# walexi/gnn.cpp

Hardware: AMD Instinct MI355X
Metric: GCN-layer edges/sec (fwd+bwd: X.W^T + normalized-adjacency SpMM + their gradients) (higher is better)
Workload: dtype f32

## Files before the change

### gnn.cpp_amd/csrc/gnnx_gemm.hip

```cpp
#include <atomic>

#include "gnnx_common.h"

using namespace gnnx;

namespace {

typedef float f32x16 __attribute__((ext_vector_type(16)));

struct GemmArgs {
    int64_t M, N, K;
    const float *A;
    int64_t lda;
    const float *B;
    int64_t ldb;
    float *C;
    int64_t ldc;
    float alpha, beta;
    int64_t k_per_split;
    float *slab;
    int64_t k_pairs;
};

template <int BM_, int BN_, int BK_, int WM_, int WN_>
struct Cfg {
    static constexpr int BM = BM_, BN = BN_, BK = BK_, WM = WM_, WN = WN_;
    static constexpr int NT = 64 * WM * WN;
    static constexpr int TM = BM / WM / 32, TN = BN / WN / 32;
    static constexpr int ld_a(bool kc) { return kc ? BM + 2 : BM + 4; }
    static constexpr int ld_b(bool kc) { return kc ? BN + 2 : BN + 4; }
    static constexpr size_t lds_bytes(bool a_kc, bool b_kc) { return sizeof(float) * 2 * BK * (ld_a(a_kc) + ld_b(b_kc)); }
    static constexpr int A_VECS = BM * BK / 4 / NT;
    static constexpr int B_VECS = BN * BK / 4 / NT;
    static_assert(A_VECS >= 1 && B_VECS >= 1, "tile too small for the thread count");
};

template <bool KC, bool VEC, int ROWS, int BK, int NT, int NV>
__device__ __forceinline__ void load_tile(float (&reg)[NV * 4], const float *base, int64_t ld, int64_t r0, int64_t rmax,
                                          int64_t k0, int64_t kmax, int tid)
{
#pragma unroll
    for (int i = 0; i < NV; i++) {
        const int idx = tid + i * NT;
        int64_t r, k;
        if constexpr (KC) {
            r = r0 + idx / (BK / 4);
            k = k0 + (idx % (BK / 4)) * 4;
            const int64_t rc = r < rmax ? r : rmax - 1;
            if constexpr (VEC) {
                const float4 v = *reinterpret_cast<const float4 *>(base + rc * ld + (k < kmax ? k : 0));
                reg[4 * i + 0] = v.x;
                reg[4 * i + 1] = v.y;
                reg[4 * i + 2] = v.z;
                reg[4 * i + 3] = v.w;
            } else {
#pragma unroll
                for (int j = 0; j < 4; j++) reg[4 * i + j] = base[rc * ld + ((k + j) < kmax ? (k + j) : 0)];
            }
        } else {
            k = k0 + idx / (ROWS / 4);
            r = r0 + (idx % (ROWS / 4)) * 4;
            const int64_t kc = k < kmax ? k : kmax - 1;
            if constexpr (VEC) {
                const float4 v = *reinterpret_cast<const float4 *>(base + kc * ld + (r < rmax ? r : 0));
                reg[4 * i + 0] = v.x;
                reg[4 * i + 1] = v.y;
                reg[4 * i + 2] = v.z;
                reg[4 * i + 3] = v.w;
            } else {
#pragma unroll
                for (int j = 0; j < 4; j++) reg[4 * i + j] = base[kc * ld + ((r + j) < rmax ? (r + j) : 0)];
            }
        }
    }
}

template <bool KC, bool MASK, int ROWS, int BK, int NT, int NV, int LD>
__device__ __forceinline__ void store_tile_impl(float *lds, const float (&reg)[NV * 4], int tid, int64_t r0, int64_t rmax,
                                                int64_t k0, int64_t kmax)
{
#pragma unroll
    for (int i = 0; i < NV; i++) {
        const int idx = tid + i * NT;
        if constexpr (KC) {
            const int r = idx / (BK / 4), k = (idx % (BK / 4)) * 4;
#pragma unroll
            for (int j = 0; j < 4; j++) {
                float v = reg[4 * i + j];
                if constexpr (MASK) v = (r0 + r < rmax && k0 + k + j < kmax) ? v : 0.f;
                lds[(k + j) * LD + r] = v;
            }
        } else {
            const int k = idx / (ROWS / 4), r = (idx % (ROWS / 4)) * 4;
            float v[4];
#pragma unroll
            for (int j = 0; j < 4; j++) {
                v[j] = reg[4 * i + j];
                if constexpr (MASK) v[j] = (k0 + k < kmax && r0 + r + j < rmax) ? v[j] : 0.f;
            }
            if constexpr (LD % 4 == 0) {
                *reinterpret_cast<float4 *>(lds + k * LD + r) = make_float4(v[0], v[1], v[2], v[3]);
            } else {
#pragma unroll
                for (int j = 0; j < 4; j++) lds[k * LD + r + j] = v[j];
            }
        }
    }
}

template <bool KC, int ROWS, int BK, int NT, int NV, int LD>
__device__ __forceinline__ void store_tile(float *lds, const float (&reg)[NV * 4], int tid, bool full, int64_t r0, int64_t rmax,
                                           int64_t k0, int64_t kmax)
{
    if (full) store_tile_impl<KC, false, ROWS, BK, NT, NV, LD>(lds, reg, tid, r0, rmax, k0, kmax);
    else store_tile_impl<KC, true, ROWS, BK, NT, NV, LD>(lds, reg, tid, r0, rmax, k0, kmax);
}

template <class C, bool A_KC, bool B_KC, bool VEC_A, bool VEC_B>
__global__ __launch_bounds__(C::NT) void gemm_kernel(GemmArgs g)
{
    constexpr int BM = C::BM, BN = C::BN, BK = C::BK, NT = C::NT, TM = C::TM, TN = C::TN;
    constexpr int LDA = C::ld_a(A_KC), LDB = C::ld_b(B_KC);
    extern __shared__ __attribute__((aligned(16))) float lds_raw[];
    const int tid = threadIdx.x;
    const int lane = tid & 63, wave = tid >> 6;
    const int wm = wave / C::WN, wn = wave % C::WN;
    const int64_t m0 = (int64_t)blockIdx.y * BM, n0 = (int64_t)blockIdx.x * BN;
    const int64_t kbeg = (int64_t)blockIdx.z * g.k_per_split;
    const int64_t kend = kbeg + g.k_per_split < g.K ? kbeg + g.k_per_split : g.K;
    const bool full_mn = m0 + BM <= g.M && n0 + BN <= g.N;

    f32x16 acc[TM][TN];
#pragma unroll
    for (int i = 0; i < TM; i++)
#pragma unroll
        for (int j = 0; j < TN; j++)
#pragma unroll
            for (int r = 0; r < 16; r++) acc[i][j][r] = 0.f;

    constexpr int STORE_AT = (BK * 3 / 4) & ~1;
    float ra[C::A_VECS * 4], rb[C::B_VECS * 4];
    int buf = 0;
    if (kbeg < kend) {
        const bool full = full_mn && kbeg + BK <= kend;
        load_tile<A_KC, VEC_A, BM, BK, NT, C::A_VECS>(ra, g.A, g.lda, m0, g.M, kbeg, kend, tid);
        load_tile<B_KC, VEC_B, BN, BK, NT, C::B_VECS>(rb, g.B, g.ldb, n0, g.N, kbeg, kend, tid);
        store_tile<A_KC, BM, BK, NT, C::A_VECS, LDA>(lds_raw, ra, tid, full, m0, g.M, kbeg, kend);
        store_tile<B_KC, BN, BK, NT, C::B_VECS, LDB>(lds_raw + 2 * BK * LDA, rb, tid, full, n0, g.N, kbeg, kend);
    }
    __syncthreads();
    for (int64_t k0 = kbeg; k0 < kend; k0 += BK) {
        const bool more = k0 + BK < kend;
// ... 103 lines not shown
        for (int i = 0; i < C::A_VECS; i++) {
            const float4 v = *reinterpret_cast<const float4 *>(abase + offa[i]);
            ra[4 * i + 0] = v.x; ra[4 * i + 1] = v.y; ra[4 * i + 2] = v.z; ra[4 * i + 3] = v.w;
        }
#pragma unroll
        for (int i = 0; i < C::B_VECS; i++) {
            const float4 v = *reinterpret_cast<const float4 *>(bbase + offb[i]);
            rb[4 * i + 0] = v.x; rb[4 * i + 1] = v.y; rb[4 * i + 2] = v.z; rb[4 * i + 3] = v.w;
        }
    };
    auto stash = [&](int b) {
        store_tile_impl<true, false, BM, BK, NT, C::A_VECS, LDA>(lds_raw + b * BK * LDA, ra, tid, 0, 0, 0, 0);
        store_tile_impl<B_KC, false, BN, BK, NT, C::B_VECS, LDB>(lds_raw + 2 * BK * LDA + b * BK * LDB, rb, tid, 0, 0, 0, 0);
    };

    f32x16 acc[TM][TN];
    constexpr int STORE_AT = (BK * 3 / 4) & ~1;
    int buf = 0;
    int64_t mt = blockIdx.y;
    if (mt < m_tiles) {
        load(mt, 0);
        stash(0);
    }
    __syncthreads();
    for (; mt < m_tiles; mt += gridDim.y) {
        const int64_t mt_next = mt + gridDim.y;
#pragma unroll
        for (int i = 0; i < TM; i++)
#pragma unroll
            for (int j = 0; j < TN; j++)
#pragma unroll
                for (int r = 0; r < 16; r++) acc[i][j][r] = 0.f;
        for (int64_t k0 = 0; k0 < g.K; k0 += BK) {
            const bool last_k = k0 + BK >= g.K;
            const bool more = !last_k || mt_next < m_tiles;
            if (more) load(last_k ? mt_next : mt, last_k ? 0 : k0 + BK);
            const float *As = lds_raw + buf * BK * LDA + wm * (BM / C::WM) + (lane & 31) + (lane >> 5) * LDA;
            const float *Bs = lds_raw + 2 * BK * LDA + buf * BK * LDB + wn * (BN / C::WN) + (lane & 31) + (lane >> 5) * LDB;
            float a[2][TM], b[2][TN];
#pragma unroll
            for (int i = 0; i < TM; i++) a[0][i] = As[32 * i];
#pragma unroll
            for (int j = 0; j < TN; j++) b[0][j] = Bs[32 * j];
#pragma unroll
            for (int kk = 0; kk < BK; kk += 2) {
                const int cur = (kk >> 1) & 1, nxt = cur ^ 1;
                if (kk + 2 < BK) {
#pragma unroll
                    for (int i = 0; i < TM; i++) a[nxt][i] = As[(kk + 2) * LDA + 32 * i];
#pragma unroll
                    for (int j = 0; j < TN; j++) b[nxt][j] = Bs[(kk + 2) * LDB + 32 * j];
                }
                __builtin_amdgcn_sched_barrier(0);
#pragma unroll
                for (int i = 0; i < TM; i++)
#pragma unroll
                    for (int j = 0; j < TN; j++)
                        acc[i][j] = __builtin_amdgcn_mfma_f32_32x32x2f32(a[cur][i], b[cur][j], acc[i][j], 0, 0, 0);
                __builtin_amdgcn_sched_barrier(0);
                if (kk == STORE_AT && more) {
                    stash(buf ^ 1);
                    __builtin_amdgcn_sched_barrier(0);
                }
            }
            __syncthreads();
            buf ^= 1;
        }
        float *cbase = g.C + mt * BM * g.ldc + n0;
#pragma unroll
        for (int i = 0; i < TM; i++)
#pragma unroll
            for (int j = 0; j < TN; j++)
#pragma unroll
                for (int r = 0; r < 16; r++)
                    (cbase + (int64_t)(i * 32 + (r & 3) + 8 * (r >> 2)) * g.ldc + j * 32)[offc] = g.alpha * acc[i][j][r];
    }
}

typedef __attribute__((address_space(3))) void gemm_lds_void_t;
typedef float gemm_f32x4 __attribute__((ext_vector_type(4)));
typedef float gemm_f32x4acc __attribute__((ext_vector_type(4)));

template <int OFF>
__device__ __forceinline__ void lds_read_b32(float &dst, uint32_t addr)
{
    static_assert(OFF >= 0 && OFF < 65536, "ds_read offset is a 16-bit unsigned immediate");
    asm volatile("ds_read_b32 %0, %1 offset:%2" : "=v"(dst) : "v"(addr), "i"(OFF) : "memory");
}

template <int WM_, int WN_>
struct DmaGeo {
    static constexpr int WM = WM_, WN = WN_, NW = WM * WN, NT = 64 * NW;
    static constexpr int BM = 64 * WM, BN = 64 * WN, BK = 32;
    static constexpr int SLOTS = BK / 4;
    static constexpr int A_ROW_BYTES = BK * 4, A_BLOCK_BYTES = 16 * A_ROW_BYTES;
    static constexpr int A_ROWS_PER_INSTR = 1024 / A_ROW_BYTES;
    static constexpr int a_xor(int row) { return (row / 2) % SLOTS; }
    static constexpr int A_STAGE_BYTES = BM * BK * 4;
    static constexpr int A_PER_WAVE = (BM / A_ROWS_PER_INSTR) / NW;
    static constexpr int rows_per_instr(int width) { return 256 / width; }
    static constexpr int KPIECE_BYTES = 272 * 4;
    static constexpr int kstage_bytes(int width) { return (BK / rows_per_instr(width)) * KPIECE_BYTES; }
    static constexpr int kgroup_off(int width, int KG)
    {
        return rows_per_instr(width) == 1 ? 4 * KG * KPIECE_BYTES : (4 * (KG % (BK / 8))) * KPIECE_BYTES + (KG / (BK / 8)) * 512;
    }
    static constexpr int krow_of(int width, int I, int lane) { return rows_per_instr(width) == 1 ? I : I + (BK / 2) * (lane / 32); }
    static constexpr int B_STAGE_BYTES = kstage_bytes(BN);
    static constexpr int B_PIECE_BYTES = KPIECE_BYTES;
    static constexpr int B_PER_WAVE = (BK / rows_per_instr(BN)) / NW;
    static constexpr int STAGES_BYTES = 2 * A_STAGE_BYTES + 2 * B_STAGE_BYTES;
    static constexpr int EP_EXTRA = A_PER_WAVE + B_PER_WAVE >= 4 ? 0 : 4 - A_PER_WAVE - B_PER_WAVE;
    static constexpr int LDS_BYTES = STAGES_BYTES + NW * EP_EXTRA * 1024;
    static_assert(A_PER_WAVE >= 1 && B_PER_WAVE >= 1, "too many wavefronts for the operand tile");
};

template <class GEO, int STAGE_ID, int KG>
__device__ __forceinline__ void dma2_read_group(float (&a)[4], float (&b)[4], const uint32_t (&ak)[GEO::SLOTS], uint32_t bk)
{
    constexpr int SA = STAGE_ID * GEO::A_STAGE_BYTES, BLK = GEO::A_BLOCK_BYTES;
    lds_read_b32<SA + 0 * BLK>(a[0], ak[KG]);
    lds_read_b32<SA + 1 * BLK>(a[1], ak[KG]);
    lds_read_b32<SA + 2 * BLK>(a[2], ak[KG]);
    lds_read_b32<SA + 3 * BLK>(a[3], ak[KG]);
    constexpr int SB = STAGE_ID * GEO::B_STAGE_BYTES + GEO::kgroup_off(GEO::BN, KG);
    lds_read_b32<SB + 0 * 64>(b[0], bk);
    lds_read_b32<SB + 1 * 64>(b[1], bk);
    lds_read_b32<SB + 2 * 64>(b[2], bk);
    lds_read_b32<SB + 3 * 64>(b[3], bk);
}

#define GNNX_DMA2_WAIT(N, set)                                                                                                   \
    asm volatile("s_waitcnt lgkmcnt(" #N ")" : "+v"(a[set][0]), "+v"(a[set][1]), "+v"(a[set][2]), "+v"(a[set][3]), "+v"(b[set][0]), \
                 "+v"(b[set][1]), "+v"(b[set][2]), "+v"(b[set][3])::"memory")
#define GNNX_DMA2_MFMA(set)                                                                                \
    _Pragma("unroll") for (int i_ = 0; i_ < 4; i_++) _Pragma("unroll") for (int j_ = 0; j_ < 4; j_++)      \
        acc[i_][j_] = __builtin_amdgcn_mfma_f32_16x16x4f32(b[set][j_], a[set][i_], acc[i_][j_], 0, 0, 0)
#define GNNX_DMA2_STEP(ST, KG, cur, nxt)                                  \
    dma2_read_group<GEO, ST, KG + 1>(a[nxt], b[nxt], ak, bk);            \
    GNNX_DMA2_WAIT(8, cur);                                               \
    GNNX_DMA2_MFMA(cur)
#define GNNX_DMA2_KTILE(ST)                                               \
    dma2_read_group<GEO, ST, 0>(a[0], b[0], ak, bk);                     \
    GNNX_DMA2_STEP(ST, 0, 0, 1);                                          \
    GNNX_DMA2_STEP(ST, 1, 1, 0);                                          \
    GNNX_DMA2_STEP(ST, 2, 0, 1);                                          \
    GNNX_DMA2_STEP(ST, 3, 1, 0);                                          \
    GNNX_DMA2_STEP(ST, 4, 0, 1);                                          \
    GNNX_DMA2_STEP(ST, 5, 1, 0);                                          \
    GNNX_DMA2_STEP(ST, 6, 0, 1);                                          \
    GNNX_DMA2_WAIT(0, 1);                                                 \
    GNNX_DMA2_MFMA(1)

__device__ __forceinline__ void dma_16B(uint32_t voff_bytes, const float *sbase, uint32_t lds_dst)
{
    uint32_t keep;
    asm volatile("s_nop 4\n\ts_mov_b32 %0, m0\n\ts_mov_b32 m0, %3\n\ts_nop 0\n\tglobal_load_lds_dwordx4 %1, %2\n\ts_mov_b32 m0, %0"
                 : "=&s"(keep) : "v"(voff_bytes), "s"(sbase), "s"(lds_dst) : "memory");
}

enum class Epi { kPlain, kReluColsum, kBnSums, kBf16, kSendSlots };

constexpr bool epi_covers_rows(Epi e) { return e == Epi::kPlain || e == Epi::kSendSlots; }

struct GemmFuse {
    const float *ymask;
    int64_t ldy;
    float *colsum_partial;
    const int32_t *slots;
};

template <int WM_, int WN_, Epi EPI, bool NG>
__global__ __launch_bounds__(64 * WM_ * WN_, 1) void gemm_dma_kernel(GemmArgs g, GemmFuse fu, int64_t m_tiles)
{
    using GEO = DmaGeo<WM_, WN_>;
    constexpr int BM = GEO::BM, BN = GEO::BN, BK = GEO::BK, NW = GEO::NW;
    constexpr int APW = GEO::A_PER_WAVE, BPW = GEO::B_PER_WAVE;
    extern __shared__ __attribute__((aligned(16))) float lds_raw[];
    const int tid = threadIdx.x;
    const int lane = tid & 63;
    const int wave = __builtin_amdgcn_readfirstlane(tid >> 6);
    const int wm = wave / GEO::WN, wn = wave % GEO::WN;
    const int q = lane >> 4, r16 = lane & 15;
    const int64_t n0 = (int64_t)blockIdx.x * BN;
    const uint32_t lds0 = (uint32_t)(uintptr_t)(gemm_lds_void_t *)lds_raw;
    constexpr uint32_t B0 = 2 * GEO::A_STAGE_BYTES;

    uint32_t offa[APW], offb[BPW], pa[APW], pb[BPW];
#pragma unroll
    for (int u = 0; u < APW; u++) {
        const int row = GEO::A_ROWS_PER_INSTR * (wave + NW * u) + lane / GEO::SLOTS;
        const int kg = (lane % GEO::SLOTS) ^ GEO::a_xor(row);
        offa[u] = (uint32_t)(row * g.lda + 4 * kg) * 4u;
        pa[u] = lds0 + (uint32_t)((wave + NW * u) * 1024);
    }
#pragma unroll
    for (int u = 0; u < BPW; u++) {
        constexpr int RPI = GEO::rows_per_instr(BN), LPR = 64 / RPI;
        const int krow = GEO::krow_of(BN, wave + NW * u, lane);
        offb[u] = (uint32_t)(krow * g.ldb + 4 * (lane % LPR)) * 4u;
        pb[u] = lds0 + B0 + (uint32_t)((wave + NW * u) * GEO::B_PIECE_BYTES);
    }
    const float *bcol = g.B + n0;
    const int64_t n_left = g.N - n0;
    const bool okb = !NG || 4 * (lane % (64 / GEO::rows_per_instr(BN))) + 4 <= n_left;
    const bool okc = !NG || wn * 64 + 4 * (lane & 15) + 4 <= n_left;
    const int64_t last_row0 = g.M - BM;
    auto row0_of = [&](int64_t mt) { return mt * BM <= last_row0 ? mt * BM : last_row0; };
    auto issue = [&](int stage, int64_t mt, int64_t k0) {
        const float *abase = g.A + row0_of(mt) * g.lda + k0;
        const float *bbase = bcol + k0 * g.ldb;
#pragma unroll
        for (int u = 0; u < (APW > BPW ? APW : BPW); u++) {
            if (u < APW) dma_16B(offa[u < APW ? u : 0], abase, pa[u < APW ? u : 0] + stage * GEO::A_STAGE_BYTES);
            if (u < BPW && okb) dma_16B(offb[u < BPW ? u : 0], bbase, pb[u < BPW ? u : 0] + stage * GEO::B_STAGE_BYTES);
        }
    };
    uint32_t ak[GEO::SLOTS];
    {
        const int row = wm * 64 + r16;
        const uint32_t xa = (uint32_t)(GEO::a_xor(row) << 4);
#pragma unroll
        for (int kg = 0; kg < GEO::SLOTS; kg++) ak[kg] = lds0 + (uint32_t)(row * GEO::A_ROW_BYTES + 4 * q) + (((uint32_t)kg << 4) ^ xa);
    }
    const uint32_t bk = lds0 + B0 + (uint32_t)(q * GEO::KPIECE_BYTES + (wn * 64 + r16) * 4);
    uint32_t ep[4];
#pragma unroll
    for (int p = 0; p < 4; p++) {
        if (p < APW) ep[p] = pa[p < APW ? p : 0] + GEO::A_STAGE_BYTES;
        else if (p - APW < BPW) ep[p] = pb[p >= APW && p - APW < BPW ? p - APW : 0] + GEO::B_STAGE_BYTES;
        else ep[p] = lds0 + (uint32_t)(GEO::STAGES_BYTES + (wave * GEO::EP_EXTRA + (p - APW - BPW)) * 1024);
    }
    const int pw = r16 >> 2;
    const uint32_t ep_wr = (pw == 0 ? ep[0] : pw == 1 ? ep[1] : pw == 2 ? ep[2] : ep[3]) + (uint32_t)((r16 & 3) * 256) +
                           (uint32_t)((q ^ (r16 & 3)) << 4);
    const uint32_t ep_rd = (uint32_t)((lane >> 4) * 256) + (uint32_t)(((lane & 15) ^ (lane >> 4)) << 4);
    constexpr int ES = EPI == Epi::kBf16 ? 2 : 4;
    const uint32_t offc = (uint32_t)((wm * 64 + (lane >> 4)) * g.ldc + wn * 64 + 4 * (lane & 15)) * (uint32_t)ES;

    gemm_f32x4acc acc[4][4];
    float a[2][4], b[2][4];
    gemm_f32x4acc csum = {0.f, 0.f, 0.f, 0.f};
    gemm_f32x4acc csq = {0.f, 0.f, 0.f, 0.f};
    gemm_f32x4acc shift4 = {0.f, 0.f, 0.f, 0.f};
    if constexpr (EPI == Epi::kBnSums)
        if (okc) shift4 = *reinterpret_cast<const gemm_f32x4acc *>(fu.ymask + n0 + wn * 64 + 4 * (lane & 15));
    const uint32_t offy = EPI == Epi::kReluColsum ? (uint32_t)((wm * 64 + (lane >> 4)) * fu.ldy + wn * 64 + 4 * (lane & 15)) * 4u : 0u;
    constexpr uint32_t SLOT_BUF = (uint32_t)BM * 32u;
    const uint32_t slot_lds = lds0 + (uint32_t)GEO::LDS_BYTES;
    const uint32_t offs = (uint32_t)((wm * 64 + (lane >> 4)) * 8 + (lane & 7)) * 4u;
    char *send_col = EPI == Epi::kSendSlots ? reinterpret_cast<char *>(fu.colsum_partial + n0 + wn * 64 + 4 * (lane & 15)) : nullptr;
    uint32_t sbuf = 0;
    int64_t mt = blockIdx.y;
    if (mt < m_tiles) issue(0, mt, 0);
    asm volatile("s_waitcnt vmcnt(0)" ::: "memory");
    __syncthreads();
    for (; mt < m_tiles; mt += gridDim.y) {
        const int64_t mt_next = mt + gridDim.y;
#pragma unroll
        for (int i = 0; i < 4; i++)
#pragma unroll
            for (int j = 0; j < 4; j++)
#pragma unroll
                for (int r = 0; r < 4; r++) acc[i][j][r] = 0.f;
        if constexpr (EPI == Epi::kSendSlots) {
            sbuf ^= SLOT_BUF;
            if (wave < BM / 32)
                dma_16B((uint32_t)lane * 16u, reinterpret_cast<const float *>(fu.slots + row0_of(mt) * 8 + wave * 256), slot_lds + sbuf + (uint32_t)wave * 1024u);
        }
        for (int64_t k0 = 0; k0 < g.K; k0 += 2 * BK) {
            const bool last = k0 + 2 * BK >= g.K;
            issue(1, mt, k0 + BK);
            GNNX_DMA2_KTILE(0);
            asm volatile("s_waitcnt vmcnt(0)" ::: "memory");
            __syncthreads();
            if (!last || mt_next < m_tiles) issue(0, last ? mt_next : mt, last ? 0 : k0 + 2 * BK);
            GNNX_DMA2_KTILE(1);
            asm volatile("s_waitcnt vmcnt(0)" ::: "memory");
            __syncthreads();
        }
        const float alpha = g.alpha;
        char *ctile = reinterpret_cast<char *>(g.C) + (row0_of(mt) * g.ldc + n0) * ES;
        const char *ytile = EPI == Epi::kReluColsum ? reinterpret_cast<const char *>(fu.ymask + row0_of(mt) * fu.ldy + n0) : nullptr;
#pragma unroll
        for (int i = 0; i < 4; i++) {
#pragma unroll
            for (int j = 0; j < 4; j++) {
                gemm_f32x4acc v = acc[i][j];
                if (alpha != 1.0f) v = v * alpha;
                asm volatile("ds_write_b128 %0, %1 offset:%2" ::"v"(ep_wr), "v"(v), "i"(64 * j) : "memory");
            }
            gemm_f32x4acc ym[4] = {};
            if constexpr (EPI == Epi::kReluColsum) {
                const char *yrow = ytile + (int64_t)(16 * i) * fu.ldy * 4;
#pragma unroll
                for (int p = 0; p < 4; p++)
                    if (okc) ym[p] = *reinterpret_cast<const gemm_f32x4acc *>(yrow + (int64_t)(4 * p) * fu.ldy * 4 + offy);
            }
            int32_t sl[4] = {-1, -1, -1, -1};
            if constexpr (EPI == Epi::kSendSlots) {
#pragma unroll
                for (int p = 0; p < 4; p++)
                    asm volatile("ds_read_b32 %0, %1 offset:%2" : "=v"(sl[p]) : "v"(slot_lds + sbuf + offs), "i"((16 * i + 4 * p) * 32) : "memory");
            }
            if constexpr (EPI == Epi::kSendSlots) asm volatile("s_waitcnt lgkmcnt(0)" : "+v"(sl[0]), "+v"(sl[1]), "+v"(sl[2]), "+v"(sl[3])::"memory");
            else asm volatile("s_waitcnt lgkmcnt(0)" ::: "memory");
            gemm_f32x4acc o[4];
#pragma unroll
            for (int p = 0; p < 4; p++) asm volatile("ds_read_b128 %0, %1" : "=v"(o[p]) : "v"(ep_rd + ep[p]) : "memory");
            asm volatile("s_waitcnt lgkmcnt(0)" : "+v"(o[0]), "+v"(o[1]), "+v"(o[2]), "+v"(o[3])::"memory");
            char *crow = ctile + (int64_t)(16 * i) * g.ldc * ES;
#pragma unroll
            for (int p = 0; p < 4; p++) {
                if constexpr (EPI == Epi::kReluColsum) {
#pragma unroll
                    for (int c = 0; c < 4; c++) o[p][c] = ym[p][c] > 0.f ? o[p][c] : 0.f;
                    csum += o[p];
                }
                if constexpr (EPI == Epi::kBnSums) {
                    const gemm_f32x4acc d = o[p] - shift4;
                    csum += d;
                    csq += d * d;
                }
                if constexpr (EPI == Epi::kBf16) {
                    union { __bf16 h[4]; uint2 u; } ob;
                    ob.h[0] = (__bf16)o[p][0];
                    ob.h[1] = (__bf16)o[p][1];
                    ob.h[2] = (__bf16)o[p][2];
                    ob.h[3] = (__bf16)o[p][3];
                    if (okc) *reinterpret_cast<uint2 *>(crow + (int64_t)(4 * p) * g.ldc * ES + offc) = ob.u;
                } else if (okc) *reinterpret_cast<gemm_f32x4acc *>(crow + (int64_t)(4 * p) * g.ldc * ES + offc) = o[p];
                if constexpr (EPI == Epi::kSendSlots) {
                    const uint64_t has = __ballot(sl[p] >= 0);
                    const int rounds = __builtin_popcountll((has | (has >> 16) | (has >> 32) | (has >> 48)) & 0xffull);
#pragma unroll 1
                    for (int k = 0; k < rounds; k += 2) {
                        const int32_t s0 = __builtin_amdgcn_ds_bpermute(((lane & 48) + k) << 2, sl[p]);
                        const int32_t s1 = __builtin_amdgcn_ds_bpermute(((lane & 48) + k + 1) << 2, sl[p]);
                        if (s0 >= 0 && okc) *reinterpret_cast<gemm_f32x4acc *>(send_col + (int64_t)s0 * fu.ldy * 4) = o[p];
                        if (s1 >= 0 && okc) *reinterpret_cast<gemm_f32x4acc *>(send_col + (int64_t)s1 * fu.ldy * 4) = o[p];
                    }
                }
            }
        }
    }
    if constexpr (EPI == Epi::kReluColsum || EPI == Epi::kBnSums) {
        gemm_f32x4acc *red = reinterpret_cast<gemm_f32x4acc *>(lds_raw);
        __syncthreads();
        red[wave * 64 + lane] = csum;
        __syncthreads();
        if (tid < BN / 4 && (!NG || 4 * tid + 4 <= n_left)) {
            const int cg = tid >> 4, c16 = tid & 15;
            gemm_f32x4acc sum = {0.f, 0.f, 0.f, 0.f};
            for (int w = 0; w < GEO::WM; w++)
                for (int lg = 0; lg < 4; lg++) sum += red[(w * GEO::WN + cg) * 64 + lg * 16 + c16];
            float *prow = fu.colsum_partial + (int64_t)blockIdx.y * (EPI == Epi::kBnSums ? 2 : 1) * g.N;
            *reinterpret_cast<gemm_f32x4acc *>(prow + n0 + 4 * tid) = sum;
        }
        if constexpr (EPI == Epi::kBnSums) {
            __syncthreads();
            red[wave * 64 + lane] = csq;
            __syncthreads();
            if (tid < BN / 4 && (!NG || 4 * tid + 4 <= n_left)) {
                const int cg = tid >> 4, c16 = tid & 15;
                gemm_f32x4acc sum = {0.f, 0.f, 0.f, 0.f};
                for (int w = 0; w < GEO::WM; w++)
                    for (int lg = 0; lg < 4; lg++) sum += red[(w * GEO::WN + cg) * 64 + lg * 16 + c16];
                *reinterpret_cast<gemm_f32x4acc *>(fu.colsum_partial + ((int64_t)blockIdx.y * 2 + 1) * g.N + n0 + 4 * tid) = sum;
            }
        }
    }
}

__global__ __launch_bounds__(256) void splitk_reduce_kernel(const float *slab, int splits, int64_t M, int64_t N, float alpha,
                                                            float beta, float *C, int64_t ldc)
{
    __shared__ float red[8][32];
    const int e = threadIdx.x & 31, q = threadIdx.x >> 5;
    const int64_t total = M * N;
    const int64_t i = (int64_t)blockIdx.x * 32 + e;
    const int per = (splits + 7) / 8;
    const int s0 = q * per, s1 = s0 + per < splits ? s0 + per : splits;
    float acc = 0.f;
    if (i < total)
        for (int s = s0; s < s1; s++) acc += slab[(int64_t)s * total + i];
    red[q][e] = acc;
    __syncthreads();
    if (q == 0 && i < total) {
        float sum = red[0][e];
#pragma unroll
        for (int k = 1; k < 8; k++) sum += red[k][e];
        const int64_t r = i / N, c = i - r * N;
        float v = alpha * sum;
        if (beta != 0.f) v += beta * C[r * ldc + c];
        C[r * ldc + c] = v;
    }
}

using CfgDefault = Cfg<128, 128, 32, 2, 2>;
using CfgWide = Cfg<128, 256, 16, 2, 4>;
using CfgTall32 = Cfg<256, 256, 32, 4, 4>;

enum TileId { kSquare, kWide, kTall32 };

TileId pick_tile(int64_t M, int64_t N)
{
    if (N <= 128) return kSquare;
    return M >= 256 ? kTall32 : kWide;
}
// ... 69 lines not shown
int launch_stream(const GemmArgs &g, bool b_kc, hipStream_t st, int64_t *rows_done)
{
    *rows_done = 0;
    const TileId tile = pick_tile(g.M, g.N);
    if (tile != kTall32 && tile != kSquare) return GNNX_OK;
    if (b_kc && tile == kTall32) return GNNX_OK;
    const TileDims t = tile_dims(g.M, g.N);
    if (g.K % t.bk != 0 || g.N % t.bn != 0) return GNNX_OK;
    const int64_t m_tiles = g.M / t.bm, cols = g.N / t.bn;
    const int64_t slots = (int64_t)kNumCU * (tile == kTall32 ? 1 : 2);
    if (m_tiles * cols < 4 * slots) return GNNX_OK;
    if ((int64_t)t.bm * g.lda >= (1ll << 30) || (int64_t)(b_kc ? t.bn : t.bk) * g.ldb >= (1ll << 30) || (int64_t)t.bm * g.ldc >= (1ll << 30))
        return GNNX_OK;
    int64_t gy = ceil_div(slots, cols);
    if (gy > m_tiles) gy = m_tiles;
    int rc;
    if (tile == kTall32) rc = launch_stream_cfg<CfgTall32, false>(g, m_tiles, gy, st);
    else rc = b_kc ? launch_stream_cfg<CfgDefault, true>(g, m_tiles, gy, st) : launch_stream_cfg<CfgDefault, false>(g, m_tiles, gy, st);
    if (rc != GNNX_OK) return rc;
    *rows_done = m_tiles * t.bm;
    return GNNX_OK;
}

template <class GEO, int STAGE_ID, int KG>
__device__ __forceinline__ void dma_tn_read_group(float (&a)[4], float (&b)[4], uint32_t ak, uint32_t bk)
{
    constexpr int SA = STAGE_ID * GEO::AT_STAGE_BYTES + GEO::kgroup_off(GEO::BM, KG);
    constexpr int SB = STAGE_ID * GEO::B_STAGE_BYTES + GEO::kgroup_off(GEO::BN, KG);
    lds_read_b32<SA + 0 * 64>(a[0], ak);
    lds_read_b32<SA + 1 * 64>(a[1], ak);
    lds_read_b32<SA + 2 * 64>(a[2], ak);
    lds_read_b32<SA + 3 * 64>(a[3], ak);
    lds_read_b32<SB + 0 * 64>(b[0], bk);
    lds_read_b32<SB + 1 * 64>(b[1], bk);
    lds_read_b32<SB + 2 * 64>(b[2], bk);
    lds_read_b32<SB + 3 * 64>(b[3], bk);
}
#define GNNX_DMATN_STEP(ST, KG, cur, nxt)                                 \
    dma_tn_read_group<GEO, ST, KG + 1>(a[nxt], b[nxt], ak, bk);           \
    GNNX_DMA2_WAIT(8, cur);                                               \
    GNNX_DMA2_MFMA(cur)
#define GNNX_DMATN_KTILE(ST)                                              \
    dma_tn_read_group<GEO, ST, 0>(a[0], b[0], ak, bk);                    \
    GNNX_DMATN_STEP(ST, 0, 0, 1);                                         \
    GNNX_DMATN_STEP(ST, 1, 1, 0);                                         \
    GNNX_DMATN_STEP(ST, 2, 0, 1);                                         \
    GNNX_DMATN_STEP(ST, 3, 1, 0);                                         \
    GNNX_DMATN_STEP(ST, 4, 0, 1);                                         \
    GNNX_DMATN_STEP(ST, 5, 1, 0);                                         \
    GNNX_DMATN_STEP(ST, 6, 0, 1);                                         \
    GNNX_DMA2_WAIT(0, 1);                                                 \
    GNNX_DMA2_MFMA(1)

template <int WM_, int WN_>
struct DmaGeoTN : DmaGeo<WM_, WN_> {
    using Base = DmaGeo<WM_, WN_>;
    static constexpr int AT_STAGE_BYTES = Base::kstage_bytes(Base::BM);
    static constexpr int AT_PIECE_BYTES = Base::KPIECE_BYTES;
    static constexpr int AT_PER_WAVE = (Base::BK / Base::rows_per_instr(Base::BM)) / Base::NW;
    static constexpr int LDS_BYTES_TN = 2 * AT_STAGE_BYTES + 2 * Base::B_STAGE_BYTES;
    static_assert(AT_PER_WAVE >= 1, "too many wavefronts for the operand tile");
};

template <int WM_, int WN_>
__global__ __launch_bounds__(64 * WM_ * WN_) void gemm_dma_tn_kernel(GemmArgs g)
{
    using GEO = DmaGeoTN<WM_, WN_>;
    constexpr int BM = GEO::BM, BN = GEO::BN, BK = GEO::BK, NW = GEO::NW;
    constexpr int APW = GEO::AT_PER_WAVE, BPW = GEO::B_PER_WAVE;
    extern __shared__ __attribute__((aligned(16))) float lds_raw[];
    const int tid = threadIdx.x;
    const int lane = tid & 63;
    const int wave = __builtin_amdgcn_readfirstlane(tid >> 6);
    const int wm = wave / GEO::WN, wn = wave % GEO::WN;
    const int q = lane >> 4, r16 = lane & 15;
    const int64_t m0 = (int64_t)blockIdx.y * BM, n0 = (int64_t)blockIdx.x * BN;
    const int64_t kbeg = (int64_t)blockIdx.z * g.k_pairs / gridDim.z * 64;
    const int64_t kend = ((int64_t)blockIdx.z + 1) * g.k_pairs / gridDim.z * 64;
    const uint32_t lds0 = (uint32_t)(uintptr_t)(gemm_lds_void_t *)lds_raw;
    constexpr uint32_t B0 = 2 * GEO::AT_STAGE_BYTES;
    uint32_t offa[APW], offb[BPW], pa[APW], pb[BPW];
#pragma unroll
    for (int u = 0; u < APW; u++) {
        constexpr int RPI = GEO::rows_per_instr(BM), LPR = 64 / RPI;
        offa[u] = (uint32_t)(GEO::krow_of(BM, wave + NW * u, lane) * g.lda + 4 * (lane % LPR)) * 4u;
        pa[u] = lds0 + (uint32_t)((wave + NW * u) * GEO::AT_PIECE_BYTES);
    }
#pragma unroll
    for (int u = 0; u < BPW; u++) {
        constexpr int RPI = GEO::rows_per_instr(BN), LPR = 64 / RPI;
        offb[u] = (uint32_t)(GEO::krow_of(BN, wave + NW * u, lane) * g.ldb + 4 * (lane % LPR)) * 4u;
        pb[u] = lds0 + B0 + (uint32_t)((wave + NW * u) * GEO::B_PIECE_BYTES);
    }
    const float *acol = g.A + m0, *bcol = g.B + n0;
    auto issue = [&](int stage, int64_t k0) {
        const float *abase = acol + k0 * g.lda;
        const float *bbase = bcol + k0 * g.ldb;
#pragma unroll
        for (int u = 0; u < (APW > BPW ? APW : BPW); u++) {
            if (u < APW) dma_16B(offa[u < APW ? u : 0], abase, pa[u < APW ? u : 0] + stage * GEO::AT_STAGE_BYTES);
            if (u < BPW) dma_16B(offb[u < BPW ? u : 0], bbase, pb[u < BPW ? u : 0] + stage * GEO::B_STAGE_BYTES);
        }
    };
    const uint32_t ak = lds0 + (uint32_t)(q * GEO::KPIECE_BYTES + (wm * 64 + r16) * 4);
    const uint32_t bk = lds0 + B0 + (uint32_t)(q * GEO::KPIECE_BYTES + (wn * 64 + r16) * 4);
    gemm_f32x4acc acc[4][4];
    float a[2][4], b[2][4];
#pragma unroll
    for (int i = 0; i < 4; i++)
#pragma unroll
        for (int j = 0; j < 4; j++)
#pragma unroll
            for (int r = 0; r < 4; r++) acc[i][j][r] = 0.f;
    if (kbeg < kend) issue(0, kbeg);
    asm volatile("s_waitcnt vmcnt(0)" ::: "memory");
    __syncthreads();
    for (int64_t k0 = kbeg; k0 < kend; k0 += 2 * BK) {
        issue(1, k0 + BK);
        GNNX_DMATN_KTILE(0);
        asm volatile("s_waitcnt vmcnt(0)" ::: "memory");
        __syncthreads();
        if (k0 + 2 * BK < kend) issue(0, k0 + 2 * BK);
        GNNX_DMATN_KTILE(1);
        asm volatile("s_waitcnt vmcnt(0)" ::: "memory");
        __syncthreads();
    }
    float *out = g.slab + (int64_t)blockIdx.z * g.M * g.N + (m0 + wm * 64 + r16) * g.N + n0 + wn * 64 + 4 * q;
#pragma unroll
    for (int i = 0; i < 4; i++)
#pragma unroll
        for (int j = 0; j < 4; j++) *reinterpret_cast<gemm_f32x4acc *>(out + (int64_t)(16 * i) * g.N + 16 * j) = acc[i][j];
}

bool dma_shape_ok(int64_t M, int64_t N, int64_t K)
{
    return K % 64 == 0 && N % 4 == 0 && N >= 64 && M >= 8 * 256;
}

template <int WM, int WN, Epi EPI, bool NG>
int launch_dma_geo(const GemmArgs &g, const GemmFuse &fu, hipStream_t st, int64_t *rows_done, int64_t *partial_rows)
{
    using GEO = DmaGeo<WM, WN>;
    constexpr int BM = GEO::BM, BN = GEO::BN, BK = GEO::BK;
    if ((int64_t)BM * g.lda >= (1ll << 28) || (int64_t)BK * g.ldb >= (1ll << 28) || (int64_t)BM * g.ldc >= (1ll << 28))
        return GNNX_OK;
    const int64_t m_tiles = epi_covers_rows(EPI) ? ceil_div(g.M, (int64_t)BM) : g.M / BM, cols = ceil_div(g.N, (int64_t)BN);
    if (g.M < BM) return GNNX_OK;
    if constexpr (EPI == Epi::kReluColsum)
        if (fu.ldy % 4 || !aligned16(fu.ymask) || (int64_t)BM * fu.ldy >= (1ll << 28)) return GNNX_OK;
    if constexpr (EPI == Epi::kBnSums)
        if (!aligned16(fu.ymask)) return GNNX_OK;
    if constexpr (EPI == Epi::kSendSlots)
        if (fu.ldy % 4 || !aligned16(fu.colsum_partial)) return GNNX_OK;
    constexpr size_t lds = GEO::LDS_BYTES + (EPI == Epi::kSendSlots ? 2 * (size_t)BM * 32 : 0);
    constexpr int wg_per_cu = 160 * 1024 / GEO::LDS_BYTES >= 2 ? 2 : 1;
    int64_t gy = ceil_div((int64_t)kNumCU * wg_per_cu, cols);
    if (gy > m_tiles) gy = m_tiles;
    static std::atomic<uint64_t> done{0};
    const int rc = lds_opt_in(&gemm_dma_kernel<WM, WN, EPI, NG>, lds, done, "gemm_dma_kernel");
    if (rc) return rc;
    hipLaunchKernelGGL((gemm_dma_kernel<WM, WN, EPI, NG>), dim3((uint32_t)cols, (uint32_t)gy, 1), dim3(GEO::NT), lds, st, g, fu, m_tiles);
    GNNX_LAUNCH_CHECK();
    if (partial_rows && (EPI == Epi::kReluColsum || EPI == Epi::kBnSums)) *partial_rows = gy;
    *rows_done = m_tiles * BM < g.M ? m_tiles * BM : g.M;
    return GNNX_OK;
}

template <int WM, int WN, int TWM, int TWN, Epi EPI>
int launch_dma_with_tail(const GemmArgs &g, const GemmFuse &fu, hipStream_t st, int64_t *rows_done)
{
    static_assert(epi_covers_rows(EPI), "the column-sum epilogues index their partials by workgroup");
    const int64_t mt256 = g.M / 256;
    GemmArgs gm = g;
    gm.M = (mt256 - mt256 % kNumCU) * 256;
    int64_t rows_main = 0;
    int rc = launch_dma_geo<WM, WN, EPI, false>(gm, fu, st, &rows_main, nullptr);
    *rows_done = rows_main;
    if (rc || rows_main != gm.M) return rc;
    GemmArgs gt = g;
    gt.A += rows_main * g.lda;
    gt.C += rows_main * g.ldc;
    gt.M = g.M - rows_main;
    GemmFuse ft = fu;
    if constexpr (EPI == Epi::kSendSlots) ft.slots += rows_main * 8;
    int64_t rows_tail = 0;
    rc = launch_dma_geo<TWM, TWN, EPI, false>(gt, ft, st, &rows_tail, nullptr);
    *rows_done = rows_main + rows_tail;
    return rc;
}

template <Epi EPI>
int launch_dma(const GemmArgs &g, const GemmFuse &fu, hipStream_t st, int64_t *rows_done, int64_t *partial_rows = nullptr)
{
    *rows_done = 0;
    if (!dma_shape_ok(g.M, g.N, g.K)) return GNNX_OK;
    if (g.lda % 4 || g.ldb % 4 || g.ldc % 4 || !aligned16(g.A) || !aligned16(g.B) || !aligned16(g.C)) return GNNX_OK;
    if constexpr (EPI == Epi::kBf16)
        if (g.alpha != 1.0f) return GNNX_OK;
    if constexpr (epi_covers_rows(EPI)) {
        const int64_t mt256 = g.M / 256, r = mt256 % kNumCU;
        if (mt256 > kNumCU && r > 0) {
            if (g.N == 256 && r <= kNumCU / 4) return launch_dma_with_tail<4, 4, 2, 2, EPI>(g, fu, st, rows_done);
            if (g.N == 256 && r <= kNumCU / 2) return launch_dma_with_tail<4, 4, 4, 2, EPI>(g, fu, st, rows_done);
            if (g.N == 128 && r <= kNumCU / 2) return launch_dma_with_tail<4, 2, 2, 2, EPI>(g, fu, st, rows_done);
        }
    }
    if (g.N % 256 == 0) return launch_dma_geo<4, 4, EPI, false>(g, fu, st, rows_done, partial_rows);
    if (g.N % 128 == 0) return launch_dma_geo<4, 2, EPI, false>(g, fu, st, rows_done, partial_rows);
    if constexpr (EPI == Epi::kSendSlots) return GNNX_OK;
    else return launch_dma_geo<4, 2, EPI, true>(g, fu, st, rows_done, partial_rows);
}

bool dma_tn_shape_ok(int64_t M, int64_t N, int64_t K) { return M % 128 == 0 && N % 128 == 0 && K % 64 == 0 && K >= 64 * 1024; }

template <int WM, int WN>
int launch_dma_tn_geo(const GemmArgs &g, int splits, hipStream_t st)
{
    using GEO = DmaGeoTN<WM, WN>;
    constexpr size_t lds = GEO::LDS_BYTES_TN;
    static std::atomic<uint64_t> done{0};
    int rc = lds_opt_in(&gemm_dma_tn_kernel<WM, WN>, lds, done, "gemm_dma_tn_kernel");
    if (rc) return rc;
    hipLaunchKernelGGL((gemm_dma_tn_kernel<WM, WN>), dim3((uint32_t)(g.N / GEO::BN), (uint32_t)(g.M / GEO::BM), (uint32_t)splits),
                       dim3(GEO::NT), lds, st, g);
    GNNX_LAUNCH_CHECK();
    return GNNX_OK;
}

int launch_dma_tn(const GemmArgs &g, int splits, hipStream_t st)
{
    if (g.M % 256 == 0 && g.N % 256 == 0) return launch_dma_tn_geo<4, 4>(g, splits, st);
    return launch_dma_tn_geo<2, 2>(g, splits, st);
}

__global__ __launch_bounds__(256) void gemm_transpose_w_kernel(const float *X, int64_t ldx, int64_t n_rows, int64_t n_cols, float *Y,
                                                                int64_t ldy)
{
    __shared__ float t[32][33];
    const int tx = threadIdx.x & 31, ty = threadIdx.x >> 5;
    const int64_t c0 = (int64_t)blockIdx.x * 32, r0 = (int64_t)blockIdx.y * 32;
    for (int k = ty; k < 32; k += 8)
        if (r0 + k < n_rows && c0 + tx < n_cols) t[k][tx] = X[(r0 + k) * ldx + c0 + tx];
    __syncthreads();
    for (int k = ty; k < 32; k += 8)
        if (c0 + k < n_cols && r0 + tx < n_rows) Y[(c0 + k) * ldy + r0 + tx] = t[tx][k];
}

int transpose_w(const float *W, int64_t ldw, int64_t N, int64_t K, float *wt, hipStream_t st)
{
    hipLaunchKernelGGL(gemm_transpose_w_kernel, dim3((uint32_t)ceil_div(K, 32), (uint32_t)ceil_div(N, 32)), dim3(256), 0, st, W, ldw, N, K, wt, N);
    GNNX_LAUNCH_CHECK();
    return GNNX_OK;
}

}

GNNX_API int gnnx_gemm_workspace(int transA, int transB, int64_t M, int64_t N, int64_t K, size_t *bytes)
{
    (void)transB;
    GNNX_REQUIRE(bytes && M >= 0 && N >= 0 && K >= 0, GNNX_ERR_INVALID_ARG, "bad arguments");
    *bytes = 0;
    if (transA && M > 0 && N > 0 && K > 0) {
        int splits = choose_splits(M, N, K);
        if (splits > 1) *bytes = sizeof(float) * (size_t)(splits + 1) * (size_t)M * (size_t)N;
    } else if (!transA && transB && dma_shape_ok(M, N, K)) {
        *bytes = sizeof(float) * (size_t)K * (size_t)N;
    }
    return GNNX_OK;
}

GNNX_API int gnnx_gemm_relu_colsum_workspace(int64_t M, int64_t N, int64_t K, size_t *bytes)
{
    (void)K;
    GNNX_REQUIRE(bytes && M >= 0 && N >= 0, GNNX_ERR_INVALID_ARG, "bad arguments");
    size_t cs = 0;
    int rc = gnnx_colsum_workspace(M > 256 ? M : 256, (int32_t)N, &cs);
    if (rc) return rc;
    *bytes = sizeof(float) * 256 * (size_t)N + cs;
    return GNNX_OK;
}

GNNX_API int gnnx_gemm_relu_colsum_f32(int64_t M, int64_t N, int64_t K, const float *d_A, int64_t lda, const float *d_B, int64_t ldb,
                                       const float *d_Ymask, int64_t ldy, float *d_C, int64_t ldc, float *d_colsum, void *d_workspace,
                                       size_t workspace_bytes, void *stream)
{
    GNNX_REQUIRE(M >= 0 && N > 0 && K > 0 && N < (1ll << 31), GNNX_ERR_INVALID_ARG, "bad sizes");
    GNNX_REQUIRE(d_colsum, GNNX_ERR_INVALID_ARG, "colsum is null");
    size_t need = 0;
    gnnx_gemm_relu_colsum_workspace(M, N, K, &need);
    GNNX_REQUIRE(d_workspace && workspace_bytes >= need, GNNX_ERR_WORKSPACE, "workspace %zu < required %zu", workspace_bytes, need);
    hipStream_t st = as_stream(stream);
    if (M == 0) {
        GNNX_HIP_CHECK(hipMemsetAsync(d_colsum, 0, sizeof(float) * (size_t)N, st));
        return GNNX_OK;
    }
    GNNX_REQUIRE(d_A && d_B && d_Ymask && d_C && lda >= K && ldb >= N && ldy >= N && ldc >= N, GNNX_ERR_INVALID_ARG, "null pointer or ld");
    float *partial = static_cast<float *>(d_workspace);
    void *cs_ws = static_cast<char *>(d_workspace) + sizeof(float) * 256 * (size_t)N;
    const size_t cs_bytes = workspace_bytes - sizeof(float) * 256 * (size_t)N;
    int64_t rows = 0, prow = 0;
    GemmArgs g{};
    g.M = M; g.N = N; g.K = K; g.A = d_A; g.lda = lda; g.B = d_B; g.ldb = ldb; g.C = d_C; g.ldc = ldc; g.alpha = 1.f; g.beta = 0.f;
    g.k_per_split = K;
    int rc = launch_dma<Epi::kReluColsum>(g, GemmFuse{d_Ymask, ldy, partial, nullptr}, st, &rows, &prow);
    if (rc) return rc;
    float beta = 0.f;
    if (rows > 0) {
// ... 299 lines not shown
```

Baseline: 1.729 billion.

## Overlap GEMM epilogue stores with next tile's MFMA k-loop in plain DMA kernel

For the plain, non-NG DMA GEMM path, the kernel now runs a software-pipelined persistent loop. Half of each output tile's accumulator rows are staged through a per-wave LDS buffer and written to global memory while the first and last k-tiles of neighbouring tiles are still issuing MFMAs. The goal is to hide the epilogue's LDS transpose and global store latency behind compute, instead of draining the pipeline between M-tiles. In exchange it adds per-wave LDS space, hand-scheduled inline asm with exec-mask tricks and sched barriers, and more register pressure, which could cost occupancy or introduce ordering bugs.

```diff
diff --git a/gnn.cpp_amd/csrc/gnnx_gemm.hip b/gnn.cpp_amd/csrc/gnnx_gemm.hip
--- a/gnn.cpp_amd/csrc/gnnx_gemm.hip
+++ b/gnn.cpp_amd/csrc/gnnx_gemm.hip
@@ -1,3 +1,4 @@
+#include <type_traits>
 #include <atomic>
 
 #include "gnnx_common.h"
@@ -407,6 +408,140 @@
     GNNX_DMA2_WAIT(0, 1);                                                 \
     GNNX_DMA2_MFMA(1)
 
+template <class GEO, int ST, int KG, int HALF>
+__device__ __forceinline__ void dma2_read_half(float (&a)[4], float (&b)[4], const uint32_t (&ak)[GEO::SLOTS], uint32_t bk)
+{
+    constexpr int SA = ST * GEO::A_STAGE_BYTES, BLK = GEO::A_BLOCK_BYTES;
+    lds_read_b32<SA + (2 * HALF) * BLK>(a[2 * HALF], ak[KG]);
+    lds_read_b32<SA + (2 * HALF + 1) * BLK>(a[2 * HALF + 1], ak[KG]);
+    constexpr int SB = ST * GEO::B_STAGE_BYTES + GEO::kgroup_off(GEO::BN, KG);
+    lds_read_b32<SB + 0 * 64>(b[0], bk);
+    lds_read_b32<SB + 1 * 64>(b[1], bk);
+    lds_read_b32<SB + 2 * 64>(b[2], bk);
+    lds_read_b32<SB + 3 * 64>(b[3], bk);
+}
+
+struct DmaStaging {
+    uint32_t wr, rd, offc;
+    int64_t ldc_bytes;
+    float alpha;
+};
+
+#define GNNX_SB() __builtin_amdgcn_sched_barrier(0)
+#define GNNX_SPLIT_MFMA(i_, j_) acc[i_][j_] = __builtin_amdgcn_mfma_f32_16x16x4f32(b[cur][j_], a[cur][i_], acc[i_][j_], 0, 0, 0)
+
+template <int SUB, int FIRST_ROW>
+__device__ __forceinline__ void dma2_store_sub(const gemm_f32x4acc &o, const DmaStaging &sg, const char *ctile)
+{
+    const char *crow = ctile + (int64_t)(FIRST_ROW + 4 * SUB) * sg.ldc_bytes;
+    asm volatile("s_nop 4\n\tglobal_store_dwordx4 %0, %1, %2\n\ts_nop 1" ::"v"(sg.offc), "v"(o), "s"(crow) : "memory");
+}
+
+template <class GEO, int ST, int S0, int T>
+__device__ __forceinline__ void dma2_split_step(gemm_f32x4acc (&acc)[4][4], float (&a)[2][4], float (&b)[2][4], const uint32_t (&ak)[GEO::SLOTS],
+                                                 uint32_t bk, gemm_f32x4acc &o, const DmaStaging &sg, const char *ctile)
+{
+    static_assert(S0 == 0 || S0 == 8, "staging runs beside one of the two halves");
+    constexpr int HALF = T / 8, cur = T & 1, nxt = cur ^ 1, r0 = 2 * HALF, r1 = 2 * HALF + 1;
+    constexpr bool STAGING = T >= S0 && T < S0 + 8;
+    constexpr bool STORE_DUE = T > S0 && T <= S0 + 8;
+    constexpr int FIRST_ROW = S0 == 8 ? 0 : 32;
+    constexpr int READS = T < 15 ? 6 : 0;
+    if constexpr (T < 15) dma2_read_half<GEO, ST, (T + 1) % 8, (T + 1) / 8>(a[nxt], b[nxt], ak, bk);
+    asm volatile("s_waitcnt lgkmcnt(%6)"
+                 : "+v"(a[cur][r0]), "+v"(a[cur][r1]), "+v"(b[cur][0]), "+v"(b[cur][1]), "+v"(b[cur][2]), "+v"(b[cur][3])
+                 : "i"(READS + (STORE_DUE ? 5 : 0))
+                 : "memory");
+    if constexpr (!STAGING && !STORE_DUE) {
+#pragma unroll
+        for (int i_ = r0; i_ <= r1; i_++)
+#pragma unroll
+            for (int j_ = 0; j_ < 4; j_++) GNNX_SPLIT_MFMA(i_, j_);
+    } else {
+        GNNX_SPLIT_MFMA(r0, 0);
+        GNNX_SB();
+        if constexpr (STORE_DUE) {
+            asm volatile("s_waitcnt lgkmcnt(%1)" : "+v"(o) : "i"(READS) : "memory");
+            dma2_store_sub<T - 1 - S0, FIRST_ROW>(o, sg, ctile);
+        }
+        if constexpr (STAGING) {
+            constexpr int n = T - S0, i = FIRST_ROW / 16 + n / 4, p = n % 4;
+            constexpr int32_t MASK = (int32_t)(0x000f000fu << (4 * p));
+            if constexpr (p == 0) {
+                if (sg.alpha != 1.0f) {
+#pragma unroll
+                    for (int j_ = 0; j_ < 4; j_++) acc[i][j_] = acc[i][j_] * sg.alpha;
+                }
+            }
+            GNNX_SB();
+#define GNNX_SPLIT_WRITE(j_)                                                                                              \
+    asm volatile("s_mov_b32 exec_lo, %3\n\ts_mov_b32 exec_hi, %3\n\tds_write_b128 %0, %1 offset:%2\n\ts_mov_b64 exec, -1" \
+                 ::"v"(sg.wr), "v"(acc[i][j_]), "i"(64 * j_), "i"(MASK) : "memory")
+            GNNX_SPLIT_WRITE(0);
+            GNNX_SB();
+            GNNX_SPLIT_MFMA(r0, 1);
+            GNNX_SB();
+            GNNX_SPLIT_WRITE(1);
+            GNNX_SB();
+            GNNX_SPLIT_MFMA(r0, 2);
+            GNNX_SB();
+            GNNX_SPLIT_WRITE(2);
+            GNNX_SB();
+            GNNX_SPLIT_MFMA(r0, 3);
+            GNNX_SB();
+            GNNX_SPLIT_WRITE(3);
+            GNNX_SB();
+#undef GNNX_SPLIT_WRITE
+            GNNX_SPLIT_MFMA(r1, 0);
+            GNNX_SB();
+            asm volatile("ds_read_b128 %0, %1" : "=v"(o) : "v"(sg.rd) : "memory");
+            GNNX_SB();
+            if constexpr (p == 3) {
+#pragma unroll
+                for (int j_ = 0; j_ < 4; j_++)
+#pragma unroll
+                    for (int r = 0; r < 4; r++) acc[i][j_][r] = 0.f;
+            }
+        } else {
+            GNNX_SB();
+            GNNX_SPLIT_MFMA(r0, 1);
+            GNNX_SPLIT_MFMA(r0, 2);
+            GNNX_SPLIT_MFMA(r0, 3);
+            GNNX_SPLIT_MFMA(r1, 0);
+        }
+        GNNX_SPLIT_MFMA(r1, 1);
+        GNNX_SPLIT_MFMA(r1, 2);
+        GNNX_SPLIT_MFMA(r1, 3);
+        if constexpr (T == 15 && STAGING) {
+            asm volatile("s_waitcnt lgkmcnt(0)" : "+v"(o)::"memory");
+            dma2_store_sub<7, FIRST_ROW>(o, sg, ctile);
+        }
+    }
+}
+
+template <class GEO, int ST, int S0>
+__device__ __forceinline__ void dma2_split_ktile(gemm_f32x4acc (&acc)[4][4], float (&a)[2][4], float (&b)[2][4], const uint32_t (&ak)[GEO::SLOTS],
+                                                  uint32_t bk, gemm_f32x4acc &o, const DmaStaging &sg, const char *ctile)
+{
+    dma2_read_half<GEO, ST, 0, 0>(a[0], b[0], ak, bk);
+    dma2_split_step<GEO, ST, S0, 0>(acc, a, b, ak, bk, o, sg, ctile);
+    dma2_split_step<GEO, ST, S0, 1>(acc, a, b, ak, bk, o, sg, ctile);
+    dma2_split_step<GEO, ST, S0, 2>(acc, a, b, ak, bk, o, sg, ctile);
+    dma2_split_step<GEO, ST, S0, 3>(acc, a, b, ak, bk, o, sg, ctile);
+    dma2_split_step<GEO, ST, S0, 4>(acc, a, b, ak, bk, o, sg, ctile);
+    dma2_split_step<GEO, ST, S0, 5>(acc, a, b, ak, bk, o, sg, ctile);
+    dma2_split_step<GEO, ST, S0, 6>(acc, a, b, ak, bk, o, sg, ctile);
+    dma2_split_step<GEO, ST, S0, 7>(acc, a, b, ak, bk, o, sg, ctile);
+    dma2_split_step<GEO, ST, S0, 8>(acc, a, b, ak, bk, o, sg, ctile);
+    dma2_split_step<GEO, ST, S0, 9>(acc, a, b, ak, bk, o, sg, ctile);
+    dma2_split_step<GEO, ST, S0, 10>(acc, a, b, ak, bk, o, sg, ctile);
+    dma2_split_step<GEO, ST, S0, 11>(acc, a, b, ak, bk, o, sg, ctile);
+    dma2_split_step<GEO, ST, S0, 12>(acc, a, b, ak, bk, o, sg, ctile);
+    dma2_split_step<GEO, ST, S0, 13>(acc, a, b, ak, bk, o, sg, ctile);
+    dma2_split_step<GEO, ST, S0, 14>(acc, a, b, ak, bk, o, sg, ctile);
+    dma2_split_step<GEO, ST, S0, 15>(acc, a, b, ak, bk, o, sg, ctile);
+}
+
 __device__ __forceinline__ void dma_16B(uint32_t voff_bytes, const float *sbase, uint32_t lds_dst)
 {
     uint32_t keep;
@@ -417,6 +552,7 @@
 enum class Epi { kPlain, kReluColsum, kBnSums, kBf16, kSendSlots };
 
 constexpr bool epi_covers_rows(Epi e) { return e == Epi::kPlain || e == Epi::kSendSlots; }
+constexpr bool gemm_dma_metered(Epi e, bool ng) { return e == Epi::kPlain && !ng; }
 
 struct GemmFuse {
     const float *ymask;
@@ -510,6 +646,73 @@
     if (mt < m_tiles) issue(0, mt, 0);
     asm volatile("s_waitcnt vmcnt(0)" ::: "memory");
     __syncthreads();
+    if constexpr (gemm_dma_metered(EPI, NG)) {
+        DmaStaging sg;
+        sg.wr = lds0 + (uint32_t)(GEO::LDS_BYTES + wave * 1024 + (r16 & 3) * 256 + ((q ^ (r16 & 3)) << 4));
+        sg.rd = lds0 + (uint32_t)(GEO::LDS_BYTES + wave * 1024) + ep_rd;
+        sg.offc = offc;
+        sg.ldc_bytes = g.ldc * ES;
+        sg.alpha = g.alpha;
+        gemm_f32x4acc o1;
+        const char *ctile_prev = nullptr;
+#pragma unroll
+        for (int i = 0; i < 4; i++)
+#pragma unroll
+            for (int j = 0; j < 4; j++)
+#pragma unroll
+                for (int r = 0; r < 4; r++) acc[i][j][r] = 0.f;
+        auto tile = [&](auto first) {
+            const int64_t mt_next = mt + gridDim.y;
+            const char *ctile = reinterpret_cast<char *>(g.C) + (row0_of(mt) * g.ldc + n0) * ES;
+            issue(1, mt, BK);
+            if constexpr (decltype(first)::value) {
+                GNNX_DMA2_KTILE(0);
+                asm volatile("s_waitcnt vmcnt(0)" ::: "memory");
+            } else {
+                dma2_split_ktile<GEO, 0, 0>(acc, a, b, ak, bk, o1, sg, ctile_prev);
+                asm volatile("s_waitcnt vmcnt(8)" ::: "memory");
+            }
+            __syncthreads();
+            for (int64_t k0 = BK; k0 + BK < g.K; k0 += 2 * BK) {
+                issue(0, mt, k0 + BK);
+                GNNX_DMA2_KTILE(1);
+                asm volatile("s_waitcnt vmcnt(0)" ::: "memory");
+                __syncthreads();
+                issue(1, mt, k0 + 2 * BK);
+                GNNX_DMA2_KTILE(0);
+                asm volatile("s_waitcnt vmcnt(0)" ::: "memory");
+                __syncthreads();
+            }
+            if (mt_next < m_tiles) issue(0, mt_next, 0);
+            dma2_split_ktile<GEO, 1, 8>(acc, a, b, ak, bk, o1, sg, ctile);
+            asm volatile("s_waitcnt vmcnt(8)" ::: "memory");
+            __syncthreads();
+            ctile_prev = ctile;
+            mt = mt_next;
+        };
+        if (mt < m_tiles) {
+            tile(std::true_type{});
+            while (mt < m_tiles) tile(std::false_type{});
+#pragma unroll
+            for (int i = 2; i < 4; i++) {
+#pragma unroll
+                for (int j = 0; j < 4; j++) {
+                    gemm_f32x4acc v = acc[i][j];
+                    if (sg.alpha != 1.0f) v = v * sg.alpha;
+                    asm volatile("ds_write_b128 %0, %1 offset:%2" ::"v"(ep_wr), "v"(v), "i"(64 * j) : "memory");
+                }
+                asm volatile("s_waitcnt lgkmcnt(0)" ::: "memory");
+                gemm_f32x4acc o[4];
+#pragma unroll
+                for (int p = 0; p < 4; p++) asm volatile("ds_read_b128 %0, %1" : "=v"(o[p]) : "v"(ep_rd + ep[p]) : "memory");
+                asm volatile("s_waitcnt lgkmcnt(0)" : "+v"(o[0]), "+v"(o[1]), "+v"(o[2]), "+v"(o[3])::"memory");
+#pragma unroll
+                for (int p = 0; p < 4; p++)
+                    *reinterpret_cast<gemm_f32x4acc *>(const_cast<char *>(ctile_prev) + (int64_t)(16 * i + 4 * p) * sg.ldc_bytes + offc) = o[p];
+            }
+        }
+        return;
+    }
     for (; mt < m_tiles; mt += gridDim.y) {
         const int64_t mt_next = mt + gridDim.y;
 #pragma unroll
@@ -885,7 +1088,8 @@
         if (!aligned16(fu.ymask)) return GNNX_OK;
     if constexpr (EPI == Epi::kSendSlots)
         if (fu.ldy % 4 || !aligned16(fu.colsum_partial)) return GNNX_OK;
-    constexpr size_t lds = GEO::LDS_BYTES + (EPI == Epi::kSendSlots ? 2 * (size_t)BM * 32 : 0);
+    constexpr size_t lds = GEO::LDS_BYTES + (EPI == Epi::kSendSlots ? 2 * (size_t)BM * 32 : 0) + (gemm_dma_metered(EPI, NG) ? (size_t)GEO::NW * 1024 : 0);
+    static_assert(lds <= 160 * 1024, "a CU's LDS");
     constexpr int wg_per_cu = 160 * 1024 / GEO::LDS_BYTES >= 2 ? 2 : 1;
     int64_t gy = ceil_div((int64_t)kNumCU * wg_per_cu, cols);
     if (gy > m_tiles) gy = m_tiles;
```

New measurement: 1.746 billion (median of 6 runs). No clear change (+1.0%).
